# nabeelre/BTSbot

Measured on AMD Instinct MI355X. Metric: alerts/sec (63×63×3 triplet + 25 meta) train+infer, 1/2/4/8 MI355X, higher is better.
Workload: dtype bf16; 1 GPU; BASELINE.json configs[1]: ConvNeXt-pico multi-modal (mm_ConvNeXt) bf16 inference, batch=1024 synthetic triplets per GPU, inputs resident in HBM, logits+scores out; per_gpu_batch=1024, global_batch=1024, precision=bf16, weights=seeded random, layer-scale ~1, parallelism=1 independent replicas, batch-sharded, no collective, pipeline_depth=3

## Files before the change

### btsbot_amd/csrc/stage0b.hip

```cpp
#include <type_traits>

#include "stage0.h"
#include "stage_regs.h"

namespace {

constexpr int C = 64, HW = 15, P = 225, CT = 2, HID = 256;
constexpr int PITCH = 2 * C + 16;
static_assert(C == StageRegs<CT>::C && PITCH == StageRegs<CT>::PITCH, "ln_regs / regs_to_map derive both from CT");
static_assert(256 * PITCH <= C * 800, "the [pixel][channel] image overlays the planar one");
constexpr int PL_ROWS = 22, PL_XQ = PL_ROWS * 8, PL_CH = 800;
constexpr int PLB = C * PL_CH;
constexpr int CHUNKB = 8192, NCH = HID / 32, NSLOT = 3;
constexpr int TW_R = 21, TW_BYTES = TW_R * C * 4 * 4 * 2;
constexpr int PF_DWB = 0, PF_LNW = C, PF_LNB = 2 * C, PF_B1 = 3 * C, PF_B2 = PF_B1 + HID, PF_FLOATS = 512;
static_assert(PF_B2 + C == PF_FLOATS, "parameter image layout");
constexpr int PARB = TW_BYTES + PF_FLOATS * 4;
constexpr int PARB_X2 = 2 * TW_BYTES + PF_FLOATS * 4;
constexpr int LNP = 4 * C + 16;
constexpr int LNIMGB = P * LNP;
static_assert(LNIMGB % 16 == 0 && PLB + CHUNKB <= LNIMGB, "ring slot 2 inside the image's tail, behind the planar image");
template <bool X2> struct S0L {
  static constexpr int PLANES = X2 ? 2 : 1;
  static constexpr int CHB = X2 ? 2 * CHUNKB : CHUNKB;
  static constexpr int OFF_RING = X2 ? PLANES * PLB : LNIMGB;
  static constexpr int OFF_SLOT2 = X2 ? OFF_RING + 2 * CHB : PLB;
  static constexpr int OFF_B1 = OFF_RING + (X2 ? NSLOT : 2) * CHB;
  static constexpr int LDS_BYTES = OFF_B1 + (HID + 3 * C) * 4;
  static __device__ __forceinline__ int slot(int s) { return s == 2 ? OFF_SLOT2 : OFF_RING + s * CHB; }
};
static_assert(S0L<false>::LDS_BYTES <= 81920, "two workgroups per CU");
static_assert(S0L<true>::LDS_BYTES <= 160 * 1024, "one workgroup per CU");
static_assert(LNIMGB <= S0L<true>::OFF_RING && LNIMGB <= S0L<false>::OFF_RING, "the fp32 image in front of ring slots 0 and 1");

#define SB_STAMP(i)                                                                \
  do {                                                                             \
    if (a.stamps != nullptr && blockIdx.x == 0 && threadIdx.x == 0) {             \
      a.stamps[i] = clock64();                                                     \
      asm volatile("s_waitcnt vmcnt(0)" ::: "memory");  \
    }                                                                              \
    if (a.wgt != nullptr && threadIdx.x == 0 && ((i) == 0 || (i) == 13))           \
      a.wgt[2 * blockIdx.x + ((i) == 13)] = wall_clock64();                        \
  } while (0)

struct __attribute__((packed, aligned(4))) f4u { float v[4]; };

template <typename T, int LOPLANE = 0, bool SAT = false>
__device__ __forceinline__ void regs_to_planar(const f32x16 (&x)[CT], unsigned char* pl, int p, int h) {
  const int y = p / HW, xx = p - y * HW;
  unsigned char* dst = pl + (xx >> 2) * PL_XQ + (y + 3) * 8 + (xx & 3) * 2 + h * 4 * PL_CH;
#pragma unroll
  for (int ct = 0; ct < CT; ++ct)
#pragma unroll
    for (int r = 0; r < 16; ++r) {
      const T hi = (T)(SAT ? __builtin_amdgcn_fmed3f(x[ct][r], -65504.0f, 65504.0f) : x[ct][r]);
      *reinterpret_cast<T*>(dst + (ct * 32 + 8 * (r >> 2) + (r & 3)) * PL_CH) = hi;
      if (LOPLANE > 0)
        *reinterpret_cast<T*>(dst + LOPLANE + (ct * 32 + 8 * (r >> 2) + (r & 3)) * PL_CH) = (T)(x[ct][r] - (float)hi);
    }
}

__device__ __forceinline__ void regs_to_tap(const f32x16 (&x)[CT], float* tap, int h) {
#pragma unroll
  for (int ct = 0; ct < CT; ++ct)
#pragma unroll
    for (int qd = 0; qd < 4; ++qd)
      *reinterpret_cast<float4*>(tap + ct * 32 + 8 * qd + 4 * h) =
          make_float4(x[ct][4 * qd], x[ct][4 * qd + 1], x[ct][4 * qd + 2], x[ct][4 * qd + 3]);
}

template <typename T, bool X2, int WPS = 2, bool KEEP = false, typename HT = T>
__global__ __launch_bounds__(256, WPS) void stage0b_kernel(Stage0Args a) {
  using frag = typename Mfma<T>::frag;
  using hfrag = typename Mfma<HT>::frag;
  constexpr bool PKG = std::is_same<HT, f16_t>::value && !X2 && !KEEP;
  static_assert(std::is_same<HT, T>::value || PKG, "a hidden type of its own: f16, inference, one operand");
  using DT = typename std::conditional<KEEP, f16_t, T>::type;
  using frag4 = typename Mfma<DT>::frag4;
  extern __shared__ __attribute__((aligned(16))) unsigned char smem[];
  unsigned char* map = smem;
  unsigned char* pl = smem;
  using L = S0L<X2>;
  constexpr int PLO = X2 ? PLB : 0;
  float* b1s = reinterpret_cast<float*>(smem + L::OFF_B1);
  float* b2s = b1s + HID;
  float* lnws = b2s + C;
  float* lnbs = lnws + C;

  const int tid = threadIdx.x, lane = tid & 63, wave = tid >> 6;
  const int lr = lane & 31, h = lane >> 5;
  const int alert = blockIdx.x;
  int pix[2];
  bool live[2];
#pragma unroll
  for (int t = 0; t < 2; ++t) {
    pix[t] = wave * 64 + t * 32 + lr;
    live[t] = pix[t] < P;
  }
  const int dj = lane & 3, dch = wave * 16 + (lane >> 2);

  SB_STAMP(0);
  frag4 tw[TW_R], twl[X2 ? TW_R : 1];
  float dwbias, lng, lnb2, b1v, b2v;
  auto load_block_params = [&](int j) {
    const Stage0Blk& bk = a.blk[j];
    const uint2* src = reinterpret_cast<const uint2*>(bk.par) + wave * 64 + lane;
#pragma unroll
    for (int r = 0; r < TW_R; ++r) tw[r] = __builtin_bit_cast(frag4, src[r * 256]);
    if (X2) {
#pragma unroll
      for (int r = 0; r < TW_R; ++r) twl[r] = __builtin_bit_cast(frag4, src[TW_BYTES / 8 + r * 256]);
    }
    const float* pf = reinterpret_cast<const float*>(bk.par + (X2 ? 2 : 1) * TW_BYTES);
    dwbias = pf[PF_DWB + dch];
    lng = pf[PF_LNW + (tid & 63)];
    lnb2 = pf[PF_LNB + (tid & 63)];
    b1v = pf[PF_B1 + tid];
    b2v = pf[PF_B2 + (tid & 63)];
  };
  load_block_params(0);
  auto zero_planar = [&]() {
    for (int i = tid; i < L::PLANES * PLB / 16; i += 256) reinterpret_cast<uint4*>(pl)[i] = make_uint4(0u, 0u, 0u, 0u);
  };
  zero_planar();
  __syncthreads();

  f32x16 x[2][CT];
  {
    const float* src = a.img + (size_t)alert * 3 * 63 * 63;
    const T* sw = reinterpret_cast<const T*>(a.stem_w);
    frag af[3][CT], afl[X2 ? 3 : 1][CT];
#pragma unroll
    for (int ci = 0; ci < 3; ++ci)
#pragma unroll
      for (int ct = 0; ct < CT; ++ct) {
        af[ci][ct] = *reinterpret_cast<const frag*>(sw + (ct * 32 + lr) * 48 + ci * 16 + h * 8);
        if (X2)
          afl[ci][ct] = *reinterpret_cast<const frag*>(reinterpret_cast<const T*>(a.stem_w_lo) + (ct * 32 + lr) * 48 + ci * 16 + h * 8);
      }
#pragma unroll
    for (int t = 0; t < 2; ++t) {
      const int pc = live[t] ? pix[t] : 0;
      const int py = pc / HW, px = pc - py * HW;
#pragma unroll
      for (int ct = 0; ct < CT; ++ct)
#pragma unroll
        for (int qd = 0; qd < 4; ++qd) {
          const float4 bv = *reinterpret_cast<const float4*>(a.stem_b + ct * 32 + 8 * qd + 4 * h);
          x[t][ct][4 * qd + 0] = bv.x;
          x[t][ct][4 * qd + 1] = bv.y;
          x[t][ct][4 * qd + 2] = bv.z;
          x[t][ct][4 * qd + 3] = bv.w;
        }
#pragma unroll
      for (int ci = 0; ci < 3; ++ci) {
        const float* r0 = src + (ci * 63 + 4 * py + 2 * h) * 63 + 4 * px;
        const f4u v0 = *reinterpret_cast<const f4u*>(r0);
        const f4u v1 = *reinterpret_cast<const f4u*>(r0 + 63);
        frag bf, bfl;
#pragma unroll
        for (int e = 0; e < 4; ++e) {
          bf[e] = (T)v0.v[e];
          bf[4 + e] = (T)v1.v[e];
          if (X2) {
            bfl[e] = (T)(v0.v[e] - (float)bf[e]);
            bfl[4 + e] = (T)(v1.v[e] - (float)bf[4 + e]);
          }
        }
#pragma unroll
        for (int ct = 0; ct < CT; ++ct) {
          if (X2) {
            x[t][ct] = Mfma<T>::m32(afl[ci][ct], bf, x[t][ct]);
            x[t][ct] = Mfma<T>::m32(af[ci][ct], bfl, x[t][ct]);
          }
          x[t][ct] = Mfma<T>::m32(af[ci][ct], bf, x[t][ct]);
        }
      }
      if (KEEP && live[t]) regs_to_tap(x[t], a.keep_stem_pre + ((size_t)alert * P + pix[t]) * C, h);
      ln_regs(x[t], a.stem_lnw, a.stem_lnb, h, x[t]);
      if (live[t]) regs_to_planar<DT, PLO, KEEP && !std::is_same<T, f16_t>::value>(x[t], pl, pix[t], h);
      if (a.tap_stem != nullptr && live[t])
        regs_to_tap(x[t], a.tap_stem + ((size_t)alert * P + pix[t]) * C, h);
    }
  }
  SB_STAMP(1);

#pragma unroll
  for (int j = 0; j < 2; ++j) {
    const Stage0Blk& bk = a.blk[j];
    SB_STAMP(2 + 5 * j);
    __syncthreads();
    b1s[tid] = b1v;
    if (tid < C) {
      b2s[tid] = b2v;
      lnws[tid] = lng;
      lnbs[tid] = lnb2;
    }

    const unsigned char* wsrc[2];
    const unsigned char* wsrcl[2];
#pragma unroll
    for (int i = 0; i < 2; ++i) {
      const int pc = wave * 2 + i;
      if (pc < 4) {
        const int m = pc * 8 + (lane >> 3);
        const int hid = (m & ~12) | ((m & 4) << 1) | ((m & 8) >> 1);
        const size_t o = (size_t)hid * (C * 2) + (((lane & 7) ^ ((m >> 1) & 7)) << 4);
        wsrc[i] = bk.w1 + o;
        wsrcl[i] = X2 ? bk.w1_lo + o : nullptr;
      } else {
        const int r = (pc - 4) * 16 + (lane >> 2);
        const size_t o = (size_t)r * (HID * 2) + (((lane & 3) ^ swz4(r)) << 4);
        wsrc[i] = bk.w2g + o;
        wsrcl[i] = X2 ? bk.w2g_lo + o : nullptr;
      }
    }
    const int wstep0 = wave < 2 ? 32 * C * 2 : 64;
    auto issue = [&](int ch) {
#pragma unroll
      for (int i = 0; i < 2; ++i)
        __builtin_amdgcn_global_load_lds((gptr_t)(wsrc[i] + (size_t)ch * wstep0),
                                         (lptr_t)(smem + L::slot(ch % NSLOT) + (wave * 2 + i) * 1024),
                                         16, 0, 0);
      if (X2) {
#pragma unroll
        for (int i = 0; i < 2; ++i)
          __builtin_amdgcn_global_load_lds((gptr_t)(wsrcl[i] + (size_t)ch * wstep0),
                                           (lptr_t)(smem + L::slot(ch % NSLOT) + CHUNKB + (wave * 2 + i) * 1024),
                                           16, 0, 0);
      }
    };
    SB_STAMP(3 + 5 * j);
// ... 221 lines not shown
#pragma unroll
              for (int r = 0; r < 8; ++r) hx[r] = hacc[t][8 * s2 + r];
              f16x2v g2[4];
              gelu_pk4(hx, g2);
              hf = __builtin_shufflevector(__builtin_shufflevector(g2[0], g2[1], 0, 1, 2, 3),
                                           __builtin_shufflevector(g2[2], g2[3], 0, 1, 2, 3), 0, 1, 2, 3, 4, 5, 6, 7);
            } else {
#pragma unroll
              for (int r = 0; r < 8; ++r) {
#ifdef S0_EXP_NOGELU
                const float gv = hacc[t][8 * s2 + r];
#else
                const float gv = gelu_for<T>(hacc[t][8 * s2 + r]);
#endif
                hf[r] = (HT)gv;
                if (X2) hfl[r] = (HT)(gv - (float)hf[r]);
              }
            }
#pragma unroll
            for (int ct = 0; ct < CT; ++ct) {
              if (X2) {
                x[t][ct] = Mfma<HT>::m32(a2l[ct][s2], hf, x[t][ct]);
                x[t][ct] = Mfma<HT>::m32(a2[ct][s2], hfl, x[t][ct]);
              }
              x[t][ct] = Mfma<HT>::m32(a2[ct][s2], hf, x[t][ct]);
            }
          }
        }
      }
      if (j == 0) {
        load_block_params(1);
#pragma unroll
        for (int t = 0; t < 2; ++t) {
          if (live[t]) regs_to_planar<DT, PLO, KEEP && !std::is_same<T, f16_t>::value>(x[t], pl, pix[t], h);
          if (KEEP && live[t]) regs_to_tap(x[t], a.keep_xin1 + ((size_t)alert * P + pix[t]) * C, h);
        }
      }
    }
    SB_STAMP(6 + 5 * j);
  }
  if (a.tap_stage != nullptr) {
#pragma unroll
    for (int t = 0; t < 2; ++t)
      if (live[t]) regs_to_tap(x[t], a.tap_stage + ((size_t)alert * P + pix[t]) * C, h);
  }

  {
    const T* dw = reinterpret_cast<const T*>(a.ds_w) + (size_t)(wave * 32 + lr) * 256 + h * 8;
    frag af[16], afl[X2 ? 16 : 1];
#pragma unroll
    for (int ks = 0; ks < 16; ++ks) af[ks] = *reinterpret_cast<const frag*>(dw + ks * 16);
    constexpr int MAPB = 256 * PITCH;
    static_assert(MAPB <= PLB && 2 * MAPB <= S0L<true>::OFF_RING, "the 16-bit [pixel][channel] image(s) in front of every ring slot");
#pragma unroll
    for (int t = 0; t < 2; ++t) {
      f32x16 xn[CT];
      ln_regs(x[t], a.ds_lnw, a.ds_lnb, h, xn);
      regs_to_map<T, X2 ? MAPB : 0>(xn, map, pix[t], h);
    }
    if (X2) {
      const T* dwl = reinterpret_cast<const T*>(a.ds_w_lo) + (size_t)(wave * 32 + lr) * 256 + h * 8;
#pragma unroll
      for (int ks = 0; ks < 16; ++ks) afl[ks] = *reinterpret_cast<const frag*>(dwl + ks * 16);
    }
    __syncthreads();
    if (KEEP) {
      unsigned char* dst = reinterpret_cast<unsigned char*>(a.keep_patches) + (size_t)alert * 49 * 4 * C * 2;
      for (int i = tid; i < 49 * 4 * 8; i += 256) {
        const int c16 = i & 7, q = (i >> 3) & 3, o = i >> 5;
        const int pin = (2 * (o / 7) + (q >> 1)) * HW + 2 * (o % 7) + (q & 1);
        *reinterpret_cast<uint4*>(dst + (size_t)(o * 4 + q) * C * 2 + 16 * c16) =
            *reinterpret_cast<const uint4*>(map + pin * PITCH + 16 * c16);
      }
    }
    SB_STAMP(12);
#pragma unroll
    for (int t = 0; t < 2; ++t) {
      const int o = t * 32 + lr;
      const bool olive = o < 49;
      const int oc = olive ? o : 0;
      const int oy = oc / 7, ox = oc - oy * 7;
      f32x16 acc;
#pragma unroll
      for (int qd = 0; qd < 4; ++qd) {
        const float4 bv = *reinterpret_cast<const float4*>(a.ds_b + wave * 32 + 8 * qd + 4 * h);
        acc[4 * qd + 0] = bv.x;
        acc[4 * qd + 1] = bv.y;
        acc[4 * qd + 2] = bv.z;
        acc[4 * qd + 3] = bv.w;
      }
#pragma unroll
      for (int ks = 0; ks < 16; ++ks) {
        const int q = ks >> 2;
        const int pin = (2 * oy + (q >> 1)) * HW + 2 * ox + (q & 1);
        const frag bf = *reinterpret_cast<const frag*>(map + pin * PITCH + (ks & 3) * 32 + h * 16);
        if (X2) {
          const frag bfl = *reinterpret_cast<const frag*>(map + MAPB + pin * PITCH + (ks & 3) * 32 + h * 16);
          acc = Mfma<T>::m32(afl[ks], bf, acc);
          acc = Mfma<T>::m32(af[ks], bfl, acc);
        }
        acc = Mfma<T>::m32(af[ks], bf, acc);
      }
      if (olive) {
        float* dst = a.out + ((size_t)alert * 49 + o) * 128 + wave * 32 + 4 * h;
#pragma unroll
        for (int qd = 0; qd < 4; ++qd)
          *reinterpret_cast<float4*>(dst + 8 * qd) =
              make_float4(acc[4 * qd], acc[4 * qd + 1], acc[4 * qd + 2], acc[4 * qd + 3]);
      }
    }
    SB_STAMP(13);
  }
}

template <typename T, bool X2>
__global__ void pack_s0par_kernel(const float* __restrict__ taps, const float* __restrict__ dw_b,
                                  const float* __restrict__ ln_w, const float* __restrict__ ln_b,
                                  const float* __restrict__ b1, const float* __restrict__ b2,
                                  const float* __restrict__ gamma, unsigned char* __restrict__ out) {
  const int idx = blockIdx.x * blockDim.x + threadIdx.x;
  constexpr int NTW = TW_R * C * 16;
  if (idx < NTW) {
    const int k = idx & 3, i = (idx >> 2) & 3, c = (idx >> 4) & (C - 1), r = idx >> 10;
    const int ky = r / 3, rb = r % 3 - 1, kx = 4 * rb + k - i + 3;
    const float w = (kx >= 0 && kx < 7) ? taps[(ky * 7 + kx) * C + c] : 0.f;
    const T wh = (T)w;
    reinterpret_cast<T*>(out)[idx] = wh;
    if (X2) reinterpret_cast<T*>(out)[NTW + idx] = (T)(w - (float)wh);
    return;
  }
  const int f = idx - NTW;
  if (f >= PF_FLOATS) return;
  float v;
  if (f < PF_LNW) v = dw_b[f - PF_DWB];
  else if (f < PF_LNB) v = ln_w[f - PF_LNW];
  else if (f < PF_B1) v = ln_b[f - PF_LNB];
  else if (f < PF_B2) v = b1[f - PF_B1];
  else v = gamma[f - PF_B2] * b2[f - PF_B2];
  reinterpret_cast<float*>(out + (X2 ? 2 : 1) * TW_BYTES)[f] = v;
}

template <typename T, bool X2 = false, int WPS = 2, bool KEEP = false, typename HT = T>
int launch_stage0b_t(const Stage0Args& a, hipStream_t st) {
  auto kern = stage0b_kernel<T, X2, WPS, KEEP, HT>;
  static DevOnce attr_set;
  static const int pad = switch_on(SW_S0_ONE_WG) && !X2 ? 90 * 1024 - S0L<X2>::LDS_BYTES : 0;
  const int LDS_BYTES = S0L<X2>::LDS_BYTES + pad;
  if (attr_set.need()) {
    HIP_TRY(hipFuncSetAttribute(reinterpret_cast<const void*>(kern),
                                hipFuncAttributeMaxDynamicSharedMemorySize, (int)LDS_BYTES));
    attr_set.done();
  }
  hipLaunchKernelGGL(kern, dim3(a.B), dim3(256), LDS_BYTES, st, a);
  LAUNCH_CHECK();
  return BTSBOT_OK;
}

}

#ifdef STAGE0B_X2_TU
int launch_stage0b_x2(const Stage0Args& a, hipStream_t st) {
// ... 67 lines not shown
```

### btsbot_amd/csrc/stage1b.hip

```cpp
#include "stage0.h"
#include "stage_regs.h"
#include <type_traits>

namespace {

constexpr int C = 128, HW = 7, PA = 49, CT = 4, HID = 512, KS1 = 8;
constexpr int CN = 256, PO = 9;
constexpr int PITCH = 2 * C + 16;
static_assert(C == StageRegs<CT>::C && PITCH == StageRegs<CT>::PITCH, "ln_regs / regs_to_map derive both from CT");
constexpr int CHUNKB = 16384, HALFB = CHUNKB / 2, NCH = HID / 32, NSLOT = 3;
constexpr int PL_ROW = 136 * 8, PL_XQ = 8 * PL_ROW, PL_AL = 2 * PL_XQ;
constexpr int OFF_PL = 2 * CHUNKB;
constexpr int LNP = 4 * C + 16;
template <int G, bool X2> struct S1L {
  static_assert(G == 2 || (G == 5 && !X2), "two planar images of five alerts do not fit LDS");
  static constexpr int NW = G == 2 ? 4 : 8, NT = 64 * NW;
  static constexpr int NPX = G * PA;
  static constexpr int NG = 8 / NW;
  static constexpr int NPIECE = 16 / NW;
  static constexpr int NCB = (G * PO + 31) / 32;
  static constexpr int MAPB = NPX * PITCH;
  static constexpr int PLB = G * PL_AL;
  static constexpr int PLANES = X2 ? 2 : 1;
  static constexpr int SLB = X2 ? 2 * HALFB : HALFB;
  static constexpr int OFF_W2X = OFF_PL + PLANES * PLB;
  static constexpr int LNB = NPX * LNP;
  static constexpr int OFF_B1 = OFF_W2X + (X2 ? 2 * SLB : 0) > LNB ? OFF_W2X + (X2 ? 2 * SLB : 0) : LNB;
  static constexpr int OFF_LNW = OFF_B1 + (HID + C) * 4;
  static constexpr int LDS_BYTES = OFF_LNW + 2 * C * 4;
  static_assert(4 * SLB <= PLANES * PLB, "W1 slots + W2 slot 0 inside the planar images");
  static_assert(LNB <= OFF_B1 && OFF_B1 % 16 == 0, "the fp32 image ends in front of the bias words");
  static_assert((X2 ? 2 : 1) * MAPB <= OFF_B1, "the [pixel][channel] image(s) in front of the bias words");
};
static_assert(S1L<2, false>::LDS_BYTES <= 75264 && S1L<2, true>::LDS_BYTES <= 160 * 1024 && S1L<5, false>::LDS_BYTES <= 160 * 1024,
              "LDS layout");
constexpr int TW_R = 21, TW_BYTES = TW_R * C * 4 * 4 * 2;
constexpr int PARB = TW_BYTES + 3 * C * 4;
constexpr int PARB_X2 = 2 * TW_BYTES + 3 * C * 4;

#define SC_STAMP(i)                                                                \
  do {                                                                             \
    if (a.stamps != nullptr && blockIdx.x == 0 && threadIdx.x == 0) a.stamps[i] = clock64(); \
    if (a.wgt != nullptr && threadIdx.x == 0 && ((i) == 0 || (i) == 13))           \
      a.wgt[2 * blockIdx.x + ((i) == 13)] = wall_clock64();                        \
  } while (0)

template <typename T, int G, int LOPLANE = 0, bool SAT = false>
__device__ __forceinline__ void regs_to_planar(const f32x16 (&x)[CT], unsigned char* pl, int p, int h) {
  const int al = G == 2 ? (p >= PA ? 1 : 0) : p / PA, pp = p - al * PA;
  const int y = pp / HW, xx = pp - y * HW;
  unsigned char* dst = pl + al * PL_AL + (xx >> 2) * PL_XQ + y * PL_ROW + (xx & 3) * 2 + h * 32;
#pragma unroll
  for (int ct = 0; ct < CT; ++ct)
#pragma unroll
    for (int r = 0; r < 16; ++r) {
      const T hi = (T)(SAT ? __builtin_amdgcn_fmed3f(x[ct][r], -65504.0f, 65504.0f) : x[ct][r]);
      *reinterpret_cast<T*>(dst + (ct * 32 + 8 * (r >> 2) + (r & 3)) * 8) = hi;
      if (LOPLANE > 0) *reinterpret_cast<T*>(dst + LOPLANE + (ct * 32 + 8 * (r >> 2) + (r & 3)) * 8) = (T)(x[ct][r] - (float)hi);
    }
}

template <typename T, bool X2, int WPS = 2, bool KEEP = false, int G = 2>
__global__ __launch_bounds__((S1L<G, X2>::NT), WPS) void stage1b_kernel(Stage1Args a) {
  using frag = typename Mfma<T>::frag;
  using DT = typename std::conditional<KEEP, f16_t, T>::type;
  using frag4 = typename Mfma<DT>::frag4;
  extern __shared__ __attribute__((aligned(16))) unsigned char smem[];
  unsigned char* pl = smem + OFF_PL;
  unsigned char* stg = smem;
  using L = S1L<G, X2>;
  static_assert(G == 2 || !KEEP, "the keeping forms hold two alerts");
  constexpr int SLB = L::SLB, NW = L::NW, NT = L::NT, NPX = L::NPX, NG = L::NG, NPIECE = L::NPIECE, PLB = L::PLB, MAPB = L::MAPB;
  constexpr int PLO = X2 ? PLB : 0;
  float* b1s = reinterpret_cast<float*>(smem + L::OFF_B1);
  float* b2s = b1s + HID;
  float* lnws = reinterpret_cast<float*>(smem + L::OFF_LNW);
  float* lnbs = lnws + C;
  auto w1slot = [&](int sl) { return pl + sl * SLB; };
  auto w2slot = [&](int sl) { return sl == 0 ? pl + 3 * SLB : (X2 ? smem + L::OFF_W2X : smem) + (sl - 1) * SLB; };

  const int tid = threadIdx.x, lane = tid & 63, wave = __builtin_amdgcn_readfirstlane(tid >> 6);
  const int lr = lane & 31, h = lane >> 5;
  const bool w1wave = wave < NW / 2;
  const int a0 = blockIdx.x * G;
  const int nal = min(G, a.B - a0);
  const int p = wave * 32 + lr;
  const bool live = p < nal * PA;
  const bool inmap = p < NPX;
  const int pm = inmap ? p : 0;
  const int lnrow = pm * LNP + h * 32;
  SC_STAMP(0);
  auto zero_pads = [&]() {
#pragma unroll
    for (int pn = 0; pn < L::PLANES; ++pn) {
      unsigned char* pb = pl + pn * PLB;
      for (int i = tid; i < 2 * G * PL_ROW / 16; i += NT) {
        const int blk = i / (PL_ROW / 16), o = i - blk * (PL_ROW / 16);
        *reinterpret_cast<uint4*>(pb + (blk >> 1) * PL_AL + (blk & 1) * PL_XQ + 7 * PL_ROW + o * 16) = make_uint4(0u, 0u, 0u, 0u);
      }
      for (int i = tid; i < G * HW * C; i += NT) {
        const int al = i / (HW * C), r = (i / C) % HW, c = i % C;
        *reinterpret_cast<unsigned short*>(pb + al * PL_AL + PL_XQ + r * PL_ROW + c * 8 + 6) = 0;
      }
    }
  };
  zero_pads();
  const float* xsrc = a.x_in + ((size_t)a0 * PA + (live ? p : 0)) * C;
  float* xscr = a.scratch + ((size_t)a0 * PA + (live ? p : 0)) * C;
  auto load_x = [&](const float* src, f32x16 (&x)[CT]) {
#pragma unroll
    for (int ct = 0; ct < CT; ++ct)
#pragma unroll
      for (int qd = 0; qd < 4; ++qd) {
        const float4 v4 = *reinterpret_cast<const float4*>(src + ct * 32 + 8 * qd + 4 * h);
        x[ct][4 * qd + 0] = live ? v4.x : 0.f;
        x[ct][4 * qd + 1] = live ? v4.y : 0.f;
        x[ct][4 * qd + 2] = live ? v4.z : 0.f;
        x[ct][4 * qd + 3] = live ? v4.w : 0.f;
      }
  };
  {
    f32x16 x0[CT];
    load_x(xsrc, x0);
    if (inmap) regs_to_planar<DT, G, PLO, KEEP && !std::is_same<T, f16_t>::value>(x0, pl, p, h);
  }
  SC_STAMP(1);

  f32x16 x[CT];
#pragma unroll
  for (int j = 0; j < 2; ++j) {
    const Stage0Blk& bk = a.blk[j];
    int ln = lane;
    asm volatile("" : "+v"(ln));
    const int dj = ln & 3, db = ln >> 2;
    const float b1v0 = bk.b1[tid], b1v1 = NT == 256 ? bk.b1[256 + tid] : 0.f;
    const float b2v = bk.gamma[tid & (C - 1)] * bk.b2[tid & (C - 1)];
    const uint2* twsrc = reinterpret_cast<const uint2*>(bk.par) + (NG * wave) * 64 + ln;
    frag4 tw[TW_R], twl[X2 ? TW_R : 1];
#pragma unroll
    for (int r = 0; r < TW_R; ++r) tw[r] = __builtin_bit_cast(frag4, twsrc[r * 512]);
    if (X2) {
#pragma unroll
      for (int r = 0; r < TW_R; ++r) twl[r] = __builtin_bit_cast(frag4, twsrc[TW_BYTES / 8 + r * 512]);
    }
    const float* pf = reinterpret_cast<const float*>(bk.par + (X2 ? 2 : 1) * TW_BYTES);
    float dwbias[NG];
#pragma unroll
    for (int gi = 0; gi < NG; ++gi) dwbias[gi] = pf[16 * (NG * wave + gi) + db];
    const float lnv = pf[C + (NT == 256 ? tid : tid & 255)];
    SC_STAMP(2 + 5 * j);
    __syncthreads();
    b1s[tid] = b1v0;
    if (NT == 256) b1s[256 + tid] = b1v1;
    if (tid < C) b2s[tid] = b2v;
    if (NT == 256 || tid < 2 * C) lnws[tid] = lnv;

    const unsigned char* wsrc[NPIECE];
    const unsigned char* wsrcl[NPIECE];
#pragma unroll
    for (int i = 0; i < NPIECE; ++i) {
      const int pc = wave * NPIECE + i;
      if (pc < 8) {
        const int m = pc * 4 + (lane >> 4);
        const int hid = (m & ~12) | ((m & 4) << 1) | ((m & 8) >> 1);
        const size_t o = (size_t)hid * (C * 2) + (((lane & 15) ^ (m & 15)) << 4);
        wsrc[i] = bk.w1 + o;
        wsrcl[i] = X2 ? bk.w1_lo + o : nullptr;
      } else {
        const int r = (pc - 8) * 16 + (lane >> 2);
        const size_t o = (size_t)r * (HID * 2) + (((lane & 3) ^ swz4(r)) << 4);
        wsrc[i] = bk.w2g + o;
        wsrcl[i] = X2 ? bk.w2g_lo + o : nullptr;
      }
    }
    const int wstep0 = w1wave ? 32 * C * 2 : 64;
    auto issue = [&](int k) {
      unsigned char* dst = (w1wave ? w1slot(k % NSLOT) : w2slot(k % NSLOT)) + (wave & (NW / 2 - 1)) * (NPIECE * 1024);
#pragma unroll
// ... 345 lines not shown
#pragma unroll
        for (int ct = 0; ct < CT; ++ct) {
          if (X2) {
            x[ct] = Mfma<T>::m32(a2l[ct][1], hf, x[ct]);
            x[ct] = Mfma<T>::m32(a2[ct][1], hfl, x[ct]);
          }
          x[ct] = Mfma<T>::m32(a2[ct][1], hf, x[ct]);
        }
        LS(7);
      };
#ifndef S1_EXP_NOLOOP
#pragma unroll 1
      for (int ch = 0; ch < NCH - 2; ch += 2) {
        step(std::false_type{}, ch, hacc[0], hacc[1]);
        step(std::false_type{}, ch + 1, hacc[1], hacc[0]);
      }
      step(std::false_type{}, NCH - 2, hacc[0], hacc[1]);
      step(std::true_type{}, NCH - 1, hacc[1], hacc[0]);
#endif
      asm volatile("s_waitcnt lgkmcnt(0)" ::: "memory");
#ifdef S1_LOOPSTAMP
      if (a.wgt != nullptr && blockIdx.x == 0 && tid == 0 && j == 0)
        for (int i = 0; i < 16; ++i) a.wgt[4096 + i] = lts[i];
#endif
      wait_vm<0>();
      if (j == 0) {
        __syncthreads();
        zero_pads();
        if (inmap) regs_to_planar<DT, G, PLO, KEEP && !std::is_same<T, f16_t>::value>(x, pl, p, h);
        if (live) {
#pragma unroll
          for (int ct = 0; ct < CT; ++ct)
#pragma unroll
            for (int qd = 0; qd < 4; ++qd)
              *reinterpret_cast<float4*>(xscr + ct * 32 + 8 * qd + 4 * h) =
                  make_float4(x[ct][4 * qd], x[ct][4 * qd + 1], x[ct][4 * qd + 2], x[ct][4 * qd + 3]);
        }
      }
    }
    SC_STAMP(6 + 5 * j);
  }
  if (a.tap_stage != nullptr && live) {
    float* tp = a.tap_stage + ((size_t)a0 * PA + p) * C;
#pragma unroll
    for (int ct = 0; ct < CT; ++ct)
#pragma unroll
      for (int qd = 0; qd < 4; ++qd)
        *reinterpret_cast<float4*>(tp + ct * 32 + 8 * qd + 4 * h) =
            make_float4(x[ct][4 * qd], x[ct][4 * qd + 1], x[ct][4 * qd + 2], x[ct][4 * qd + 3]);
  }

  {
    __syncthreads();
    {
      f32x16 xn[CT];
      ln_regs(x, a.ds_lnw, a.ds_lnb, h, xn);
      if (inmap) regs_to_map<T, X2 ? MAPB : 0>(xn, stg, p, h);
    }
    constexpr int KSD = 4 * C / 16, RING = X2 ? 8 : 16, NSTEP = NG * KSD, NCB = L::NCB;
    const frag* wsrc = reinterpret_cast<const frag*>(a.ds_w) + lane;
    auto fsrc = [&](int stp) {
      return wsrc + (size_t)((wave + NW * (stp >> 5)) * KSD + (stp & (KSD - 1))) * (X2 ? 128 : 64);
    };
    frag wq[RING], wql[X2 ? RING : 1];
#pragma unroll
    for (int i = 0; i < RING; ++i) {
      wq[i] = *fsrc(i);
      if (X2) wql[i] = fsrc(i)[64];
    }
    __syncthreads();
    if (KEEP) {
      unsigned char* dst = reinterpret_cast<unsigned char*>(a.keep_patches) + (size_t)a0 * PO * 4 * C * 2;
      for (int i = tid; i < nal * PO * 4 * 16; i += NT) {
        const int c16 = i & 15, q = (i >> 4) & 3, o2 = i >> 6;
        const int g2 = o2 / PO, oo2 = o2 - g2 * PO;
        const int pin2 = g2 * PA + (2 * (oo2 / 3) + (q >> 1)) * HW + 2 * (oo2 % 3) + (q & 1);
        *reinterpret_cast<uint4*>(dst + (size_t)(o2 * 4 + q) * C * 2 + 16 * c16) =
            *reinterpret_cast<const uint4*>(stg + pin2 * PITCH + 16 * c16);
      }
    }
    SC_STAMP(12);
    int pin0[NCB];
#pragma unroll
    for (int cb = 0; cb < NCB; ++cb) {
      const int o = cb * 32 + lr, oc = o < G * PO ? o : 0;
      const int g = oc / PO, oo = oc - g * PO;
      const int oy = oo / 3, ox = oo - oy * 3;
      pin0[cb] = g * PA + 2 * oy * HW + 2 * ox;
    }
    f32x16 acc[NCB];
    constexpr int RPT = KSD / RING;
#ifdef S1_EXP_NODS
#pragma unroll 1
    for (int rd = 0; rd < 0; ++rd) {
#else
#pragma unroll 1
    for (int rd = 0; rd < NSTEP / RING; ++rd) {
#endif
      const int cot = wave + NW * (rd / RPT);
      if (rd % RPT == 0) {
#pragma unroll
        for (int qd = 0; qd < 4; ++qd) {
          const float4 bv = *reinterpret_cast<const float4*>(a.ds_b + cot * 32 + 8 * qd + 4 * h);
#pragma unroll
          for (int cb = 0; cb < NCB; ++cb) {
            acc[cb][4 * qd + 0] = bv.x;
            acc[cb][4 * qd + 1] = bv.y;
            acc[cb][4 * qd + 2] = bv.z;
            acc[cb][4 * qd + 3] = bv.w;
          }
        }
      }
#pragma unroll
      for (int i = 0; i < RING; ++i) {
        const int stp = rd * RING + i, ks = stp & (KSD - 1);
        const int q = ks >> 3;
#pragma unroll
        for (int cb = 0; cb < NCB; ++cb) {
          const int pin = pin0[cb] + (q >> 1) * HW + (q & 1);
          const frag bf = *reinterpret_cast<const frag*>(stg + pin * PITCH + (ks & 7) * 32 + h * 16);
          if (X2) {
            const frag bfl = *reinterpret_cast<const frag*>(stg + MAPB + pin * PITCH + (ks & 7) * 32 + h * 16);
            acc[cb] = Mfma<T>::m32(wql[i], bf, acc[cb]);
            acc[cb] = Mfma<T>::m32(wq[i], bfl, acc[cb]);
          }
          acc[cb] = Mfma<T>::m32(wq[i], bf, acc[cb]);
        }
        if (stp + RING < NSTEP) {
          wq[i] = *fsrc(stp + RING);
          if (X2) wql[i] = fsrc(stp + RING)[64];
        }
      }
      if (rd % RPT == RPT - 1) {
#pragma unroll
        for (int cb = 0; cb < NCB; ++cb) {
          const int o = cb * 32 + lr;
          if (o >= nal * PO) continue;
          float* dst = a.out + ((size_t)a0 * PO + o) * CN + cot * 32 + 4 * h;
#pragma unroll
          for (int qd = 0; qd < 4; ++qd)
            *reinterpret_cast<float4*>(dst + 8 * qd) =
                make_float4(acc[cb][4 * qd], acc[cb][4 * qd + 1], acc[cb][4 * qd + 2], acc[cb][4 * qd + 3]);
        }
      }
    }
    SC_STAMP(13);
  }
}

template <typename T, bool X2>
__global__ void pack_s1par_kernel(const float* __restrict__ taps, const float* __restrict__ dw_b,
                                  const float* __restrict__ ln_w, const float* __restrict__ ln_b,
                                  unsigned char* __restrict__ out) {
  const int idx = blockIdx.x * blockDim.x + threadIdx.x;
  constexpr int NTW = TW_R * C * 16;
  if (idx < NTW) {
    const int k = idx & 3, i = (idx >> 2) & 3, c = (idx >> 4) & (C - 1), r = idx / (16 * C);
    const int ky = r / 3, rb = r % 3 - 1, kx = 4 * rb + k - i + 3;
    const float w = (kx >= 0 && kx < 7) ? taps[(ky * 7 + kx) * C + c] : 0.f;
    const T wh = (T)w;
    reinterpret_cast<T*>(out)[idx] = wh;
    if (X2) reinterpret_cast<T*>(out)[NTW + idx] = (T)(w - (float)wh);
    return;
  }
  const int f = idx - NTW;
  if (f >= 3 * C) return;
  float v;
  if (f < C) v = dw_b[f];
  else if (f < 2 * C) v = ln_w[f - C];
  else v = ln_b[f - 2 * C];
  reinterpret_cast<float*>(out + (X2 ? 2 : 1) * TW_BYTES)[f] = v;
}

template <typename T, bool X2 = false>
__global__ void pack_frag32_kernel(const float* __restrict__ w, T* __restrict__ out, int rows, int cin) {
  const long i = (long)blockIdx.x * blockDim.x + threadIdx.x;
  const int K = 4 * cin;
  if (i >= (long)rows * K) return;
  const int j = (int)(i & 7), l = (int)((i >> 3) & 63);
  const long fs = i >> 9;
  const int ksteps = K / 16;
  const int sk = (int)(fs % ksteps), tile = (int)(fs / ksteps);
  const int row = 32 * tile + (l & 31), k = 16 * sk + 8 * (l >> 5) + j;
  const int q = k / cin, c = k - q * cin;
  const float v = w[((long)row * cin + c) * 4 + q];
  const T vh = (T)v;
  if (X2) {
    out[fs * 1024 + l * 8 + j] = vh;
    out[fs * 1024 + 512 + l * 8 + j] = (T)(v - (float)vh);
  } else {
    out[i] = vh;
  }
}

template <typename T, bool X2 = false, int WPS = 2, bool KEEP = false, int G = 2>
int launch_stage1b_t(const Stage1Args& a, hipStream_t st) {
  auto kern = stage1b_kernel<T, X2, WPS, KEEP, G>;
  using L = S1L<G, X2>;
// ... 110 lines not shown
```

### btsbot_amd/csrc/stage_regs.h

```cpp
#pragma once
#include "mfma.h"

template <int CT> struct StageRegs {
  static constexpr int C = 32 * CT;
  static constexpr int PITCH = 64 * CT + 16;
};

template <int N> __device__ __forceinline__ void wait_vm() {
  asm volatile("s_waitcnt vmcnt(%0)" ::"n"(N) : "memory");
}
__device__ __forceinline__ int swz4(int row) {
  return (4 - ((row >> 2) & 3)) & 3;
}
template <int CT>
__device__ __forceinline__ void ln_regs(const f32x16 (&x)[CT], const float* __restrict__ w,
                                        const float* __restrict__ b, int h, f32x16 (&y)[CT]) {
  constexpr int C = StageRegs<CT>::C;
  float s = 0.f;
#pragma unroll
  for (int ct = 0; ct < CT; ++ct)
#pragma unroll
    for (int r = 0; r < 16; ++r) s += x[ct][r];
  s += __shfl_xor(s, 32, 64);
  const float mean = s * (1.0f / C);
  float q = 0.f;
#pragma unroll
  for (int ct = 0; ct < CT; ++ct)
#pragma unroll
    for (int r = 0; r < 16; ++r) {
      const float d = x[ct][r] - mean;
      q += d * d;
    }
  q += __shfl_xor(q, 32, 64);
  const float rstd = rsqrtf(q * (1.0f / C) + LN_EPS);
#pragma unroll
  for (int ct = 0; ct < CT; ++ct)
#pragma unroll
    for (int qd = 0; qd < 4; ++qd) {
      const int c = ct * 32 + 8 * qd + 4 * h;
      const float4 wv = *reinterpret_cast<const float4*>(w + c);
      const float4 bv = *reinterpret_cast<const float4*>(b + c);
      y[ct][4 * qd + 0] = (x[ct][4 * qd + 0] - mean) * rstd * wv.x + bv.x;
      y[ct][4 * qd + 1] = (x[ct][4 * qd + 1] - mean) * rstd * wv.y + bv.y;
      y[ct][4 * qd + 2] = (x[ct][4 * qd + 2] - mean) * rstd * wv.z + bv.z;
      y[ct][4 * qd + 3] = (x[ct][4 * qd + 3] - mean) * rstd * wv.w + bv.w;
    }
}

template <typename T, int LOPLANE = 0, int CT>
__device__ __forceinline__ void regs_to_map(const f32x16 (&x)[CT], unsigned char* map, int p, int h) {
  constexpr int PITCH = StageRegs<CT>::PITCH;
  typedef T T4 __attribute__((ext_vector_type(4)));
#pragma unroll
  for (int ct = 0; ct < CT; ++ct)
#pragma unroll
    for (int qd = 0; qd < 4; ++qd) {
      T4 v, w;
#pragma unroll
      for (int e = 0; e < 4; ++e) {
        v[e] = (T)x[ct][4 * qd + e];
        if (LOPLANE > 0) w[e] = (T)(x[ct][4 * qd + e] - (float)v[e]);
      }
      *reinterpret_cast<T4*>(map + p * PITCH + (ct * 32 + 8 * qd + 4 * h) * 2) = v;
      if (LOPLANE > 0) *reinterpret_cast<T4*>(map + LOPLANE + p * PITCH + (ct * 32 + 8 * qd + 4 * h) * 2) = w;
    }
}
```

Before: 4.169 million alerts/s.

## Stage LN/bias params in LDS and software-pipeline downsample B-fragment reads

Moves the downsample and stem LayerNorm weights and biases into LDS, loaded early alongside the stem image and stem weights, so the LN and bias reads no longer hit global memory on the critical path. The downsample GEMM loops in stage0b and stage1b now prefetch B fragments two k-steps ahead through a 4-deep register ring, separated by sched barriers. In stage1b the LN-to-map write is fused per channel tile after the weight prefetch, and a full __syncthreads is replaced by an lgkmcnt wait plus s_barrier. The cost is extra LDS bytes and more register pressure, which could hurt occupancy.

```diff
diff --git a/btsbot_amd/csrc/stage0b.hip b/btsbot_amd/csrc/stage0b.hip
--- a/btsbot_amd/csrc/stage0b.hip
+++ b/btsbot_amd/csrc/stage0b.hip
@@ -26,7 +26,8 @@
   static constexpr int OFF_RING = X2 ? PLANES * PLB : LNIMGB;
   static constexpr int OFF_SLOT2 = X2 ? OFF_RING + 2 * CHB : PLB;
   static constexpr int OFF_B1 = OFF_RING + (X2 ? NSLOT : 2) * CHB;
-  static constexpr int LDS_BYTES = OFF_B1 + (HID + 3 * C) * 4;
+  static constexpr int OFF_DSC = OFF_B1 + (HID + 3 * C) * 4;
+  static constexpr int LDS_BYTES = OFF_DSC + 7 * C * 4;
   static __device__ __forceinline__ int slot(int s) { return s == 2 ? OFF_SLOT2 : OFF_RING + s * CHB; }
 };
 static_assert(S0L<false>::LDS_BYTES <= 81920, "two workgroups per CU");
@@ -86,6 +87,7 @@
   float* b2s = b1s + HID;
   float* lnws = b2s + C;
   float* lnbs = lnws + C;
+  float* dscs = reinterpret_cast<float*>(smem + L::OFF_DSC);
 
   const int tid = threadIdx.x, lane = tid & 63, wave = tid >> 6;
   const int lr = lane & 31, h = lane >> 5;
@@ -100,6 +102,36 @@
   const int dj = lane & 3, dch = wave * 16 + (lane >> 2);
 
   SB_STAMP(0);
+  f4u iq[2][3][2];
+  {
+    const float* src = a.img + (size_t)alert * 3 * 63 * 63;
+#pragma unroll
+    for (int t = 0; t < 2; ++t) {
+      const int pc = live[t] ? pix[t] : 0;
+      const int py = pc / HW, px = pc - py * HW;
+#pragma unroll
+      for (int ci = 0; ci < 3; ++ci) {
+        const float* r0 = src + (ci * 63 + 4 * py + 2 * h) * 63 + 4 * px;
+        iq[t][ci][0] = *reinterpret_cast<const f4u*>(r0);
+        iq[t][ci][1] = *reinterpret_cast<const f4u*>(r0 + 63);
+      }
+    }
+  }
+  const float dscv = tid < C ? a.ds_lnw[tid] : tid < 2 * C ? a.ds_lnb[tid - C] : a.ds_b[tid - 2 * C];
+  const float stcv = tid < C ? a.stem_b[tid] : tid < 2 * C ? a.stem_lnw[tid - C] : tid < 3 * C ? a.stem_lnb[tid - 2 * C] : 0.f;
+  frag saf[3][CT], safl[X2 ? 3 : 1][CT];
+  {
+    const T* sw = reinterpret_cast<const T*>(a.stem_w);
+#pragma unroll
+    for (int ci = 0; ci < 3; ++ci)
+#pragma unroll
+      for (int ct = 0; ct < CT; ++ct) {
+        saf[ci][ct] = *reinterpret_cast<const frag*>(sw + (ct * 32 + lr) * 48 + ci * 16 + h * 8);
+        if (X2)
+          safl[ci][ct] = *reinterpret_cast<const frag*>(reinterpret_cast<const T*>(a.stem_w_lo) + (ct * 32 + lr) * 48 + ci * 16 + h * 8);
+      }
+  }
+  __builtin_amdgcn_sched_barrier(0);
   frag4 tw[TW_R], twl[X2 ? TW_R : 1];
   float dwbias, lng, lnb2, b1v, b2v;
   auto load_block_params = [&](int j) {
@@ -123,40 +155,29 @@
     for (int i = tid; i < L::PLANES * PLB / 16; i += 256) reinterpret_cast<uint4*>(pl)[i] = make_uint4(0u, 0u, 0u, 0u);
   };
   zero_planar();
+  dscs[tid] = dscv;
+  if (tid < 3 * C) dscs[4 * C + tid] = stcv;
   __syncthreads();
 
   f32x16 x[2][CT];
   {
-    const float* src = a.img + (size_t)alert * 3 * 63 * 63;
-    const T* sw = reinterpret_cast<const T*>(a.stem_w);
-    frag af[3][CT], afl[X2 ? 3 : 1][CT];
-#pragma unroll
-    for (int ci = 0; ci < 3; ++ci)
-#pragma unroll
-      for (int ct = 0; ct < CT; ++ct) {
-        af[ci][ct] = *reinterpret_cast<const frag*>(sw + (ct * 32 + lr) * 48 + ci * 16 + h * 8);
-        if (X2)
-          afl[ci][ct] = *reinterpret_cast<const frag*>(reinterpret_cast<const T*>(a.stem_w_lo) + (ct * 32 + lr) * 48 + ci * 16 + h * 8);
-      }
+    const float* stbs = dscs + 4 * C;
 #pragma unroll
     for (int t = 0; t < 2; ++t) {
-      const int pc = live[t] ? pix[t] : 0;
-      const int py = pc / HW, px = pc - py * HW;
 #pragma unroll
       for (int ct = 0; ct < CT; ++ct)
 #pragma unroll
         for (int qd = 0; qd < 4; ++qd) {
-          const float4 bv = *reinterpret_cast<const float4*>(a.stem_b + ct * 32 + 8 * qd + 4 * h);
-          x[t][ct][4 * qd + 0] = bv.x;
-          x[t][ct][4 * qd + 1] = bv.y;
-          x[t][ct][4 * qd + 2] = bv.z;
-          x[t][ct][4 * qd + 3] = bv.w;
+          const f32x4 bv = lds_f32x4(stbs + ct * 32 + 8 * qd + 4 * h);
+          x[t][ct][4 * qd + 0] = bv[0];
+          x[t][ct][4 * qd + 1] = bv[1];
+          x[t][ct][4 * qd + 2] = bv[2];
+          x[t][ct][4 * qd + 3] = bv[3];
         }
 #pragma unroll
       for (int ci = 0; ci < 3; ++ci) {
-        const float* r0 = src + (ci * 63 + 4 * py + 2 * h) * 63 + 4 * px;
-        const f4u v0 = *reinterpret_cast<const f4u*>(r0);
-        const f4u v1 = *reinterpret_cast<const f4u*>(r0 + 63);
+        const f4u v0 = iq[t][ci][0];
+        const f4u v1 = iq[t][ci][1];
         frag bf, bfl;
 #pragma unroll
         for (int e = 0; e < 4; ++e) {
@@ -170,14 +191,14 @@
 #pragma unroll
         for (int ct = 0; ct < CT; ++ct) {
           if (X2) {
-            x[t][ct] = Mfma<T>::m32(afl[ci][ct], bf, x[t][ct]);
-            x[t][ct] = Mfma<T>::m32(af[ci][ct], bfl, x[t][ct]);
-          }
-          x[t][ct] = Mfma<T>::m32(af[ci][ct], bf, x[t][ct]);
+            x[t][ct] = Mfma<T>::m32(safl[ci][ct], bf, x[t][ct]);
+            x[t][ct] = Mfma<T>::m32(saf[ci][ct], bfl, x[t][ct]);
+          }
+          x[t][ct] = Mfma<T>::m32(saf[ci][ct], bf, x[t][ct]);
         }
       }
       if (KEEP && live[t]) regs_to_tap(x[t], a.keep_stem_pre + ((size_t)alert * P + pix[t]) * C, h);
-      ln_regs(x[t], a.stem_lnw, a.stem_lnb, h, x[t]);
+      ln_regs<true>(x[t], stbs + C, stbs + 2 * C, h, x[t]);
       if (live[t]) regs_to_planar<DT, PLO, KEEP && !std::is_same<T, f16_t>::value>(x[t], pl, pix[t], h);
       if (a.tap_stem != nullptr && live[t])
         regs_to_tap(x[t], a.tap_stem + ((size_t)alert * P + pix[t]) * C, h);
@@ -505,10 +526,13 @@
     for (int ks = 0; ks < 16; ++ks) af[ks] = *reinterpret_cast<const frag*>(dw + ks * 16);
     constexpr int MAPB = 256 * PITCH;
     static_assert(MAPB <= PLB && 2 * MAPB <= S0L<true>::OFF_RING, "the 16-bit [pixel][channel] image(s) in front of every ring slot");
+    int lt = tid;
+    asm volatile("" : "+v"(lt));
+    const int ht = (lt >> 5) & 1, lrt = lt & 31;
 #pragma unroll
     for (int t = 0; t < 2; ++t) {
       f32x16 xn[CT];
-      ln_regs(x[t], a.ds_lnw, a.ds_lnb, h, xn);
+      ln_regs<true>(x[t], dscs, dscs + C, ht, xn);
       regs_to_map<T, X2 ? MAPB : 0>(xn, map, pix[t], h);
     }
     if (X2) {
@@ -516,7 +540,8 @@
 #pragma unroll
       for (int ks = 0; ks < 16; ++ks) afl[ks] = *reinterpret_cast<const frag*>(dwl + ks * 16);
     }
-    __syncthreads();
+    asm volatile("s_waitcnt lgkmcnt(0)" ::: "memory");
+    __builtin_amdgcn_s_barrier();
     if (KEEP) {
       unsigned char* dst = reinterpret_cast<unsigned char*>(a.keep_patches) + (size_t)alert * 49 * 4 * C * 2;
       for (int i = tid; i < 49 * 4 * 8; i += 256) {
@@ -527,39 +552,62 @@
       }
     }
     SB_STAMP(12);
+    const unsigned char* bsrc[2];
+    f32x16 acc[2];
 #pragma unroll
     for (int t = 0; t < 2; ++t) {
-      const int o = t * 32 + lr;
-      const bool olive = o < 49;
-      const int oc = olive ? o : 0;
+      const int o = t * 32 + lrt, oc = o < 49 ? o : 0;
       const int oy = oc / 7, ox = oc - oy * 7;
-      f32x16 acc;
-#pragma unroll
-      for (int qd = 0; qd < 4; ++qd) {
-        const float4 bv = *reinterpret_cast<const float4*>(a.ds_b + wave * 32 + 8 * qd + 4 * h);
-        acc[4 * qd + 0] = bv.x;
-        acc[4 * qd + 1] = bv.y;
-        acc[4 * qd + 2] = bv.z;
-        acc[4 * qd + 3] = bv.w;
-      }
-#pragma unroll
-      for (int ks = 0; ks < 16; ++ks) {
-        const int q = ks >> 2;
-        const int pin = (2 * oy + (q >> 1)) * HW + 2 * ox + (q & 1);
-        const frag bf = *reinterpret_cast<const frag*>(map + pin * PITCH + (ks & 3) * 32 + h * 16);
+      bsrc[t] = map + (2 * oy * HW + 2 * ox) * PITCH + ht * 16;
+    }
+#pragma unroll
+    for (int qd = 0; qd < 4; ++qd) {
+      const f32x4 bv = lds_f32x4(dscs + 2 * C + wave * 32 + 8 * qd + 4 * ht);
+#pragma unroll
+      for (int t = 0; t < 2; ++t)
+#pragma unroll
+        for (int e = 0; e < 4; ++e) acc[t][4 * qd + e] = bv[e];
+    }
+    frag bq[4][2], bql[X2 ? 4 : 1][X2 ? 2 : 1];
+    auto read_b = [&](int ks, int set) {
+      const int q = ks >> 2;
+      const int ofs = ((q >> 1) * HW + (q & 1)) * PITCH + (ks & 3) * 32;
+#pragma unroll
+      for (int t = 0; t < 2; ++t) {
+        bq[set][t] = *reinterpret_cast<const frag*>(bsrc[t] + ofs);
+        if (X2) bql[X2 ? set : 0][X2 ? t : 0] = *reinterpret_cast<const frag*>(bsrc[t] + MAPB + ofs);
+      }
+    };
+    read_b(0, 0);
+    read_b(1, 1);
+#pragma unroll
+    for (int ks = 0; ks < 16; ++ks) {
+#pragma unroll
+      for (int t = 0; t < 2; ++t) {
+        asm volatile("" : "+v"(bq[ks & 3][t]));
+        if (X2) asm volatile("" : "+v"(bql[X2 ? ks & 3 : 0][X2 ? t : 0]));
+      }
+      if (ks + 2 < 16) read_b(ks + 2, (ks + 2) & 3);
+      __builtin_amdgcn_sched_barrier(0);
+#pragma unroll
+      for (int t = 0; t < 2; ++t) {
         if (X2) {
-          const frag bfl = *reinterpret_cast<const frag*>(map + MAPB + pin * PITCH + (ks & 3) * 32 + h * 16);
-          acc = Mfma<T>::m32(afl[ks], bf, acc);
-          acc = Mfma<T>::m32(af[ks], bfl, acc);
-        }
-        acc = Mfma<T>::m32(af[ks], bf, acc);
-      }
-      if (olive) {
-        float* dst = a.out + ((size_t)alert * 49 + o) * 128 + wave * 32 + 4 * h;
+          acc[t] = Mfma<T>::m32(afl[ks], bq[ks & 3][t], acc[t]);
+          acc[t] = Mfma<T>::m32(af[ks], bql[X2 ? ks & 3 : 0][X2 ? t : 0], acc[t]);
+        }
+        acc[t] = Mfma<T>::m32(af[ks], bq[ks & 3][t], acc[t]);
+      }
+      __builtin_amdgcn_sched_barrier(0);
+    }
+#pragma unroll
+    for (int t = 0; t < 2; ++t) {
+      const int o = t * 32 + lrt;
+      if (o < 49) {
+        float* dst = a.out + ((size_t)alert * 49 + o) * 128 + wave * 32 + 4 * ht;
 #pragma unroll
         for (int qd = 0; qd < 4; ++qd)
           *reinterpret_cast<float4*>(dst + 8 * qd) =
-              make_float4(acc[4 * qd], acc[4 * qd + 1], acc[4 * qd + 2], acc[4 * qd + 3]);
+              make_float4(acc[t][4 * qd], acc[t][4 * qd + 1], acc[t][4 * qd + 2], acc[t][4 * qd + 3]);
       }
     }
     SB_STAMP(13);
diff --git a/btsbot_amd/csrc/stage1b.hip b/btsbot_amd/csrc/stage1b.hip
--- a/btsbot_amd/csrc/stage1b.hip
+++ b/btsbot_amd/csrc/stage1b.hip
@@ -27,7 +27,8 @@
   static constexpr int LNB = NPX * LNP;
   static constexpr int OFF_B1 = OFF_W2X + (X2 ? 2 * SLB : 0) > LNB ? OFF_W2X + (X2 ? 2 * SLB : 0) : LNB;
   static constexpr int OFF_LNW = OFF_B1 + (HID + C) * 4;
-  static constexpr int LDS_BYTES = OFF_LNW + 2 * C * 4;
+  static constexpr int OFF_DSC = OFF_LNW + 2 * C * 4;
+  static constexpr int LDS_BYTES = OFF_DSC + (2 * C + CN) * 4;
   static_assert(4 * SLB <= PLANES * PLB, "W1 slots + W2 slot 0 inside the planar images");
   static_assert(LNB <= OFF_B1 && OFF_B1 % 16 == 0, "the fp32 image ends in front of the bias words");
   static_assert((X2 ? 2 : 1) * MAPB <= OFF_B1, "the [pixel][channel] image(s) in front of the bias words");
@@ -76,6 +77,7 @@
   float* b2s = b1s + HID;
   float* lnws = reinterpret_cast<float*>(smem + L::OFF_LNW);
   float* lnbs = lnws + C;
+  float* dscs = reinterpret_cast<float*>(smem + L::OFF_DSC);
   auto w1slot = [&](int sl) { return pl + sl * SLB; };
   auto w2slot = [&](int sl) { return sl == 0 ? pl + 3 * SLB : (X2 ? smem + L::OFF_W2X : smem) + (sl - 1) * SLB; };
 
@@ -104,6 +106,13 @@
       }
     }
   };
+  constexpr int NDSC = (2 * C + CN) / NT;
+  float dscv[NDSC];
+#pragma unroll
+  for (int i = 0; i < NDSC; ++i) {
+    const int f = tid + i * NT;
+    dscv[i] = f < C ? a.ds_lnw[f] : f < 2 * C ? a.ds_lnb[f - C] : a.ds_b[f - 2 * C];
+  }
   zero_pads();
   const float* xsrc = a.x_in + ((size_t)a0 * PA + (live ? p : 0)) * C;
   float* xscr = a.scratch + ((size_t)a0 * PA + (live ? p : 0)) * C;
@@ -124,6 +133,8 @@
     load_x(xsrc, x0);
     if (inmap) regs_to_planar<DT, G, PLO, KEEP && !std::is_same<T, f16_t>::value>(x0, pl, p, h);
   }
+#pragma unroll
+  for (int i = 0; i < NDSC; ++i) dscs[tid + i * NT] = dscv[i];
   SC_STAMP(1);
 
   f32x16 x[CT];
@@ -575,11 +586,6 @@
 
   {
     __syncthreads();
-    {
-      f32x16 xn[CT];
-      ln_regs(x, a.ds_lnw, a.ds_lnb, h, xn);
-      if (inmap) regs_to_map<T, X2 ? MAPB : 0>(xn, stg, p, h);
-    }
     constexpr int KSD = 4 * C / 16, RING = X2 ? 8 : 16, NSTEP = NG * KSD, NCB = L::NCB;
     const frag* wsrc = reinterpret_cast<const frag*>(a.ds_w) + lane;
     auto fsrc = [&](int stp) {
@@ -591,7 +597,14 @@
       wq[i] = *fsrc(i);
       if (X2) wql[i] = fsrc(i)[64];
     }
-    __syncthreads();
+    __builtin_amdgcn_sched_barrier(0);
+    static_assert(NW * 32 * PITCH <= L::OFF_B1, "the rows of the slots beyond the image lie in dead bytes");
+    ln_regs<true>(x, dscs, dscs + C, h, x, [&](int ct) {
+      if (X2 && !inmap) return;
+      regs_to_map_ct<T, X2 ? MAPB : 0>(x, stg, p, h, ct);
+    });
+    asm volatile("s_waitcnt lgkmcnt(0)" ::: "memory");
+    __builtin_amdgcn_s_barrier();
     if (KEEP) {
       unsigned char* dst = reinterpret_cast<unsigned char*>(a.keep_patches) + (size_t)a0 * PO * 4 * C * 2;
       for (int i = tid; i < nal * PO * 4 * 16; i += NT) {
@@ -603,56 +616,63 @@
       }
     }
     SC_STAMP(12);
-    int pin0[NCB];
+    const unsigned char* bsrc[NCB];
 #pragma unroll
     for (int cb = 0; cb < NCB; ++cb) {
       const int o = cb * 32 + lr, oc = o < G * PO ? o : 0;
       const int g = oc / PO, oo = oc - g * PO;
       const int oy = oo / 3, ox = oo - oy * 3;
-      pin0[cb] = g * PA + 2 * oy * HW + 2 * ox;
+      bsrc[cb] = stg + (g * PA + 2 * oy * HW + 2 * ox) * PITCH + h * 16;
     }
     f32x16 acc[NCB];
-    constexpr int RPT = KSD / RING;
-#ifdef S1_EXP_NODS
-#pragma unroll 1
-    for (int rd = 0; rd < 0; ++rd) {
-#else
-#pragma unroll 1
-    for (int rd = 0; rd < NSTEP / RING; ++rd) {
-#endif
+    constexpr int RPT = KSD / RING, NRD = NSTEP / RING;
+    static_assert(RING % 8 == 0 && KSD % RING == 0, "a round stays inside a tile and starts at a tap's first k-step");
+    frag bq[4][NCB], bql[X2 ? 4 : 1][X2 ? NCB : 1];
+    auto read_b = [&](int stp, int set) {
+      const int ks = stp & (KSD - 1), q = ks >> 3;
+      const int ofs = ((q >> 1) * HW + (q & 1)) * PITCH + (ks & 7) * 32;
+#pragma unroll
+      for (int cb = 0; cb < NCB; ++cb) {
+        bq[set][cb] = *reinterpret_cast<const frag*>(bsrc[cb] + ofs);
+        if (X2) bql[X2 ? set : 0][X2 ? cb : 0] = *reinterpret_cast<const frag*>(bsrc[cb] + MAPB + ofs);
+      }
+    };
+    auto round = [&](auto last_c, int rd) {
+      constexpr bool LAST = decltype(last_c)::value;
       const int cot = wave + NW * (rd / RPT);
       if (rd % RPT == 0) {
 #pragma unroll
         for (int qd = 0; qd < 4; ++qd) {
-          const float4 bv = *reinterpret_cast<const float4*>(a.ds_b + cot * 32 + 8 * qd + 4 * h);
-#pragma unroll
-          for (int cb = 0; cb < NCB; ++cb) {
-            acc[cb][4 * qd + 0] = bv.x;
-            acc[cb][4 * qd + 1] = bv.y;
-            acc[cb][4 * qd + 2] = bv.z;
-            acc[cb][4 * qd + 3] = bv.w;
-          }
+          const f32x4 bv = lds_f32x4(dscs + 2 * C + cot * 32 + 8 * qd + 4 * h);
+#pragma unroll
+          for (int cb = 0; cb < NCB; ++cb)
+#pragma unroll
+            for (int e = 0; e < 4; ++e) acc[cb][4 * qd + e] = bv[e];
         }
       }
 #pragma unroll
       for (int i = 0; i < RING; ++i) {
-        const int stp = rd * RING + i, ks = stp & (KSD - 1);
-        const int q = ks >> 3;
+        const int stp = rd * RING + i;
 #pragma unroll
         for (int cb = 0; cb < NCB; ++cb) {
-          const int pin = pin0[cb] + (q >> 1) * HW + (q & 1);
-          const frag bf = *reinterpret_cast<const frag*>(stg + pin * PITCH + (ks & 7) * 32 + h * 16);
+          asm volatile("" : "+v"(bq[i & 3][cb]));
+          if (X2) asm volatile("" : "+v"(bql[X2 ? i & 3 : 0][X2 ? cb : 0]));
+        }
+        if (!LAST || i + 2 < RING) read_b(stp + 2, (i + 2) & 3);
+        __builtin_amdgcn_sched_barrier(0);
+#pragma unroll
+        for (int cb = 0; cb < NCB; ++cb) {
           if (X2) {
-            const frag bfl = *reinterpret_cast<const frag*>(stg + MAPB + pin * PITCH + (ks & 7) * 32 + h * 16);
-            acc[cb] = Mfma<T>::m32(wql[i], bf, acc[cb]);
-            acc[cb] = Mfma<T>::m32(wq[i], bfl, acc[cb]);
-          }
-          acc[cb] = Mfma<T>::m32(wq[i], bf, acc[cb]);
-        }
-        if (stp + RING < NSTEP) {
+            acc[cb] = Mfma<T>::m32(wql[i], bq[i & 3][cb], acc[cb]);
+            acc[cb] = Mfma<T>::m32(wq[i], bql[X2 ? i & 3 : 0][X2 ? cb : 0], acc[cb]);
+          }
+          acc[cb] = Mfma<T>::m32(wq[i], bq[i & 3][cb], acc[cb]);
+        }
+        if (!LAST) {
           wq[i] = *fsrc(stp + RING);
           if (X2) wql[i] = fsrc(stp + RING)[64];
         }
+        __builtin_amdgcn_sched_barrier(0);
       }
       if (rd % RPT == RPT - 1) {
 #pragma unroll
@@ -666,7 +686,14 @@
                 make_float4(acc[cb][4 * qd], acc[cb][4 * qd + 1], acc[cb][4 * qd + 2], acc[cb][4 * qd + 3]);
         }
       }
-    }
+    };
+#ifndef S1_EXP_NODS
+    read_b(0, 0);
+    read_b(1, 1);
+#pragma unroll 1
+    for (int rd = 0; rd < NRD - 1; ++rd) round(std::false_type{}, rd);
+    round(std::true_type{}, NRD - 1);
+#endif
     SC_STAMP(13);
   }
 }
diff --git a/btsbot_amd/csrc/stage_regs.h b/btsbot_amd/csrc/stage_regs.h
--- a/btsbot_amd/csrc/stage_regs.h
+++ b/btsbot_amd/csrc/stage_regs.h
@@ -12,10 +12,29 @@
 __device__ __forceinline__ int swz4(int row) {
   return (4 - ((row >> 2) & 3)) & 3;
 }
-template <int CT>
+__device__ __forceinline__ f32x4 lds_f32x4(const float* q) {
+  return __builtin_bit_cast(f32x4, *reinterpret_cast<const bf16x8*>(q));
+}
+struct LnNoSink {
+  __device__ __forceinline__ void operator()(int) const {}
+};
+template <bool LDSW = false, int CT, typename F = LnNoSink>
 __device__ __forceinline__ void ln_regs(const f32x16 (&x)[CT], const float* __restrict__ w,
-                                        const float* __restrict__ b, int h, f32x16 (&y)[CT]) {
+                                        const float* __restrict__ b, int h, f32x16 (&y)[CT], F done = F()) {
   constexpr int C = StageRegs<CT>::C;
+  f32x4 wq[LDSW ? 2 : 1][4], bq[LDSW ? 2 : 1][4];
+  auto read_pair = [&](int ct0) {
+#pragma unroll
+    for (int k = 0; k < 2; ++k)
+#pragma unroll
+      for (int qd = 0; qd < 4; ++qd) {
+        if (ct0 + k >= CT) continue;
+        wq[LDSW ? k : 0][qd] = lds_f32x4(w + (ct0 + k) * 32 + 8 * qd + 4 * h);
+        bq[LDSW ? k : 0][qd] = lds_f32x4(b + (ct0 + k) * 32 + 8 * qd + 4 * h);
+      }
+    __builtin_amdgcn_sched_barrier(0);
+  };
+  if (LDSW) read_pair(0);
   float s = 0.f;
 #pragma unroll
   for (int ct = 0; ct < CT; ++ct)
@@ -34,25 +53,37 @@
   q += __shfl_xor(q, 32, 64);
   const float rstd = rsqrtf(q * (1.0f / C) + LN_EPS);
 #pragma unroll
-  for (int ct = 0; ct < CT; ++ct)
+  for (int ct = 0; ct < CT; ++ct) {
+    if (LDSW && ct > 0 && ct % 2 == 0) {
+      __builtin_amdgcn_sched_barrier(0);
+      read_pair(ct);
+    }
 #pragma unroll
     for (int qd = 0; qd < 4; ++qd) {
       const int c = ct * 32 + 8 * qd + 4 * h;
-      const float4 wv = *reinterpret_cast<const float4*>(w + c);
-      const float4 bv = *reinterpret_cast<const float4*>(b + c);
+      float4 wv, bv;
+      if (LDSW) {
+        const f32x4 w4 = wq[LDSW ? ct & 1 : 0][qd], b4 = bq[LDSW ? ct & 1 : 0][qd];
+        wv = make_float4(w4[0], w4[1], w4[2], w4[3]);
+        bv = make_float4(b4[0], b4[1], b4[2], b4[3]);
+      } else {
+        wv = *reinterpret_cast<const float4*>(w + c);
+        bv = *reinterpret_cast<const float4*>(b + c);
+      }
       y[ct][4 * qd + 0] = (x[ct][4 * qd + 0] - mean) * rstd * wv.x + bv.x;
       y[ct][4 * qd + 1] = (x[ct][4 * qd + 1] - mean) * rstd * wv.y + bv.y;
       y[ct][4 * qd + 2] = (x[ct][4 * qd + 2] - mean) * rstd * wv.z + bv.z;
       y[ct][4 * qd + 3] = (x[ct][4 * qd + 3] - mean) * rstd * wv.w + bv.w;
     }
+    done(ct);
+  }
 }
 
-template <typename T, int LOPLANE = 0, int CT>
-__device__ __forceinline__ void regs_to_map(const f32x16 (&x)[CT], unsigned char* map, int p, int h) {
+template <typename T, int LOPLANE, int CT>
+__device__ __forceinline__ void regs_to_map_ct(const f32x16 (&x)[CT], unsigned char* map, int p, int h, int ct) {
   constexpr int PITCH = StageRegs<CT>::PITCH;
   typedef T T4 __attribute__((ext_vector_type(4)));
-#pragma unroll
-  for (int ct = 0; ct < CT; ++ct)
+  {
 #pragma unroll
     for (int qd = 0; qd < 4; ++qd) {
       T4 v, w;
@@ -64,4 +95,10 @@
       *reinterpret_cast<T4*>(map + p * PITCH + (ct * 32 + 8 * qd + 4 * h) * 2) = v;
       if (LOPLANE > 0) *reinterpret_cast<T4*>(map + LOPLANE + p * PITCH + (ct * 32 + 8 * qd + 4 * h) * 2) = w;
     }
+  }
 }
+template <typename T, int LOPLANE = 0, int CT>
+__device__ __forceinline__ void regs_to_map(const f32x16 (&x)[CT], unsigned char* map, int p, int h) {
+#pragma unroll
+  for (int ct = 0; ct < CT; ++ct) regs_to_map_ct<T, LOPLANE>(x, map, p, h, ct);
+}
```

Result: faster. 4.267 million alerts/s (median of 6 runs) (+2.3%).
